# gman90/lime

Hardware: AMD Instinct MI355X
Metric: intervals/sec for pairwise intersect+merge at 1/2/4/8 GPUs; % of HBM peak GB/s (higher is better)
Workload: dtype u32

## Files before the change

### lime_amd/csrc/intersect.hip

```cpp
#include "common.hpp"

namespace lime {

struct PairsPlan {
    lime_ctx *ctx;
    const lime_set *A, *B;
    int64_t threshold;
    int64_t tp;
    bool filtered;
    int64_t a_own, b_own;
    int64_t nt0, nt1;
    uint32_t *olo = nullptr, *ocnt = nullptr;
    uint64_t *toff = nullptr;
    uint32_t *win = nullptr;
    uint32_t *tseg = nullptr;
    int64_t total = 0;
    int tpf = 1;
    const lime_set *A_out = nullptr;
    lime_set *W = nullptr;
    int64_t reach = -1;
};

void intersect_free(PairsPlan *pl);

namespace {

constexpr int IB = 256;
constexpr int OPT = 4;
constexpr int OT = IB * OPT;
constexpr int WCAP = 4096;
constexpr int64_t SBLK = 131072;

typedef uint32_t u32x4 __attribute__((ext_vector_type(4)));

struct StreamArgs {
    const uint32_t *ogs, *oge, *orow;
    const uint32_t *pgs, *pge, *prow;
    const uint32_t *ogs_o, *oge_o, *pgs_o, *pge_o;
    int64_t no, np;
    uint32_t lo_off;
    int zw_skip;
    int64_t reach;
    int64_t tile0;
    int64_t owner0;
};

__device__ __forceinline__ void owner_keys(uint32_t og, uint32_t oe, uint32_t lo_off, int64_t tp,
                                           int64_t &lo_key, int64_t &hi_key) {
    lo_key = (int64_t)og + lo_off;
    hi_key = (int64_t)oe - tp + 1;
}

using dev::wave_lower_bound;

__device__ __forceinline__ uint32_t contig_off(const uint32_t *__restrict__ off, int32_t nc,
                                               uint32_t g) {
    int64_t c = dev::upper_bound(off, 0, (int64_t)nc, g) - 1;
    return off[c < 0 ? 0 : c];
}

__device__ __forceinline__ void wave_lower_bound2(const uint32_t *__restrict__ a, int64_t n,
                                                  int64_t key0, int64_t key1, int64_t &r0,
                                                  int64_t &r1) {
    int64_t lo0 = 0, hi0 = n, lo1 = 0, hi1 = n;
    const int lane = dev::lane_id();
    while (hi0 - lo0 > 64 || hi1 - lo1 > 64) {
        const int64_t st0 = (hi0 - lo0 + 64) / 65, st1 = (hi1 - lo1 + 64) / 65;
        const int64_t i0 = lo0 + st0 * (lane + 1) - 1, i1 = lo1 + st1 * (lane + 1) - 1;
        const bool a0 = hi0 - lo0 > 64 && i0 < hi0;
        const bool a1 = hi1 - lo1 > 64 && i1 < hi1;
        const uint32_t v0 = a0 ? a[i0] : 0u, v1 = a1 ? a[i1] : 0u;
        if (hi0 - lo0 > 64) {
            const int c = __popcll(__ballot(a0 && (int64_t)v0 < key0));
            const int64_t nlo = c == 0 ? lo0 : lo0 + st0 * c;
            hi0 = c == 64 ? hi0 : min(hi0, lo0 + st0 * (c + 1) - 1);
            lo0 = nlo;
        }
        if (hi1 - lo1 > 64) {
            const int c = __popcll(__ballot(a1 && (int64_t)v1 < key1));
            const int64_t nlo = c == 0 ? lo1 : lo1 + st1 * c;
            hi1 = c == 64 ? hi1 : min(hi1, lo1 + st1 * (c + 1) - 1);
            lo1 = nlo;
        }
    }
    const int64_t j0 = lo0 + lane, j1 = lo1 + lane;
    const bool b0 = j0 < hi0, b1 = j1 < hi1;
    const uint32_t v0 = b0 ? a[j0] : 0u, v1 = b1 ? a[j1] : 0u;
    r0 = lo0 + __popcll(__ballot(b0 && (int64_t)v0 < key0));
    r1 = lo1 + __popcll(__ballot(b1 && (int64_t)v1 < key1));
}

__global__ __launch_bounds__(IB) void k_windows(StreamArgs sa, int64_t tp, int64_t ntiles,
                                                uint32_t *__restrict__ win,
                                                const uint32_t *__restrict__ off, int32_t nc,
                                                uint32_t *__restrict__ tseg) {
    const int64_t t = (int64_t)blockIdx.x * (IB / 64) + threadIdx.x / 64;
    if (t >= ntiles) return;
    const int lane = dev::lane_id();
    const int64_t o0 = t * OT;
    const int64_t o1 = min(o0 + OT, sa.no);
    int64_t hmax = INT64_MIN;
    for (int64_t j = o0 + lane; j < o1; j += 64) hmax = max(hmax, (int64_t)sa.oge[j] - tp + 1);
    hmax = dev::wave_reduce_max(hmax);
    const int64_t lkey = (int64_t)sa.ogs[o0] + sa.lo_off;
    const int64_t lkey_last = (int64_t)sa.ogs[o1 - 1] + sa.lo_off;
    if (hmax < lkey_last) hmax = lkey_last;
    int64_t lo, hi;
    wave_lower_bound2(sa.pgs, sa.np, lkey, hmax, lo, hi);
    if (lane == 0) {
        win[2 * (sa.tile0 + t)] = (uint32_t)lo;
        win[2 * (sa.tile0 + t) + 1] = (uint32_t)hi;
    }
    if (tseg) {
        const uint32_t g0 = sa.ogs_o[o0], g1 = sa.ogs_o[o1 - 1];
        uint32_t a, b;
        if (nc <= 64) {
            const uint32_t v = lane < nc ? off[lane] : 0xffffffffu;
            const int c0 = __popcll(__ballot(lane < nc && v <= g0)) - 1;
            const int c1 = __popcll(__ballot(lane < nc && v <= g1)) - 1;
            a = off[c0 < 0 ? 0 : c0];
            b = off[c1 < 0 ? 0 : c1];
        } else {
            a = contig_off(off, nc, g0);
            b = contig_off(off, nc, g1);
        }
        if (lane == 0) tseg[sa.tile0 + t] = a == b ? a : 0xffffffffu;
    }
}

__global__ __launch_bounds__(256) void k_windows_lane(StreamArgs sa, int64_t tp, int64_t ntiles,
                                                      int64_t owmax, uint32_t *__restrict__ win,
                                                      const uint32_t *__restrict__ off, int32_t nc,
                                                      uint32_t *__restrict__ tseg) {
    const int64_t t = (int64_t)blockIdx.x * 256 + threadIdx.x;
    if (t >= ntiles) return;
    const int64_t o0 = t * OT;
    const int64_t o1 = min(o0 + OT, sa.no);
    const uint32_t g0 = sa.ogs[o0], g1 = sa.ogs[o1 - 1];
    const int64_t lkey = (int64_t)g0 + sa.lo_off;
    int64_t hkey = (int64_t)g1 + owmax - tp + 1;
    const int64_t lkey_last = (int64_t)g1 + sa.lo_off;
    if (hkey < lkey_last) hkey = lkey_last;
    int64_t bl = 0, bh = 0;
    const int64_t n = sa.np;
    for (int64_t step = n > 0 ? (int64_t)1 << (63 - __builtin_clzll((uint64_t)n)) : 0; step > 0;
         step >>= 1) {
        const uint32_t vl = bl + step <= n ? sa.pgs[bl + step - 1] : 0xffffffffu;
        const uint32_t vh = bh + step <= n ? sa.pgs[bh + step - 1] : 0xffffffffu;
        if (bl + step <= n && (int64_t)vl < lkey) bl += step;
        if (bh + step <= n && (int64_t)vh < hkey) bh += step;
    }
    win[2 * (sa.tile0 + t)] = (uint32_t)bl;
    win[2 * (sa.tile0 + t) + 1] = (uint32_t)bh;
    if (tseg) {
        const uint32_t a = contig_off(off, nc, sa.ogs_o[o0]), b = contig_off(off, nc, sa.ogs_o[o1 - 1]);
        tseg[sa.tile0 + t] = a == b ? a : 0xffffffffu;
    }
}

template <bool FILTER, bool OFFS>
__global__ __launch_bounds__(IB) void k_count(StreamArgs sa, int64_t tp, int64_t threshold,
                                              const uint32_t *__restrict__ win,
                                              uint32_t *__restrict__ olo,
                                              uint32_t *__restrict__ ocnt,
                                              uint64_t *__restrict__ tcnt,
                                              uint32_t *__restrict__ oflow) {
    __shared__ uint32_t wgs[WCAP];
    __shared__ uint64_t red[IB / 64];
    __shared__ uint32_t scratch[IB / 64 + 1];
    const int64_t t = blockIdx.x;
    const int64_t o0 = t * OT;
    const int64_t o1 = min(o0 + OT, sa.no);
    const uint32_t wlo = win[2 * (sa.tile0 + t)], whi = win[2 * (sa.tile0 + t) + 1];
    const int64_t wlen = (int64_t)whi - wlo;
    const bool in_lds = wlen <= WCAP;
    constexpr int WPT = WCAP / IB;
    uint32_t wv[WPT];
    if (in_lds && wlen > 0) {
#pragma unroll
        for (int k = 0; k < WPT; ++k)
            wv[k] = sa.pgs[wlo + min((int64_t)(k * IB + threadIdx.x), wlen - 1)];
    }
    uint32_t ogv[OPT], oev[OPT];
    static_assert(OPT == 4, "owner loads are one 16-B vector per thread");
    if (o1 - o0 == OT) {
        const uint4 g4 = reinterpret_cast<const uint4 *>(sa.ogs + o0)[threadIdx.x];
        const uint4 e4 = reinterpret_cast<const uint4 *>(sa.oge + o0)[threadIdx.x];
        ogv[0] = g4.x, ogv[1] = g4.y, ogv[2] = g4.z, ogv[3] = g4.w;
        oev[0] = e4.x, oev[1] = e4.y, oev[2] = e4.z, oev[3] = e4.w;
    } else {
#pragma unroll
        for (int k = 0; k < OPT; ++k) {
            const int64_t j = o0 + threadIdx.x * OPT + k;
            ogv[k] = j < o1 ? sa.ogs[j] : 0u;
            oev[k] = j < o1 ? sa.oge[j] : 0u;
        }
    }
    if (in_lds && wlen > 0) {
#pragma unroll
        for (int k = 0; k < WPT; ++k)
            if (k * IB + (int)threadIdx.x < wlen) wgs[k * IB + threadIdx.x] = wv[k];
    }
    __syncthreads();
    int64_t lkv[OPT], hkv[OPT], lov[OPT], hiv[OPT];
#pragma unroll
    for (int k = 0; k < OPT; ++k) owner_keys(ogv[k], oev[k], sa.lo_off, tp, lkv[k], hkv[k]);
    if (in_lds) {
        int64_t key[2 * OPT];
        int b[2 * OPT];
#pragma unroll
        for (int k = 0; k < OPT; ++k) {
            key[k] = lkv[k];
            key[OPT + k] = hkv[k];
        }
        dev::lds_lower_bounds(wgs, (int)wlen, key, b);
#pragma unroll
        for (int k = 0; k < OPT; ++k) {
            lov[k] = wlo + b[k];
            hiv[k] = hkv[k] > lkv[k] ? wlo + b[OPT + k] : lov[k];
        }
    } else {
#pragma unroll
        for (int k = 0; k < OPT; ++k) {
            lov[k] = dev::lower_bound(sa.pgs, (int64_t)wlo, (int64_t)whi, lkv[k]);
            hiv[k] = hkv[k] > lkv[k] ? dev::lower_bound(sa.pgs, lov[k], (int64_t)whi, hkv[k])
                                     : lov[k];
        }
    }
    uint32_t cv[OPT];
    uint64_t csum = 0;
#pragma unroll
    for (int k = 0; k < OPT; ++k) {
        const int64_t j = o0 + threadIdx.x * OPT + k;
        cv[k] = 0;
        if (j >= o1) continue;
        const uint32_t og = ogv[k];
        int64_t lo = lov[k], hi = hiv[k];
        const bool keep0 = sa.reach > 0 && og == 0 && (int64_t)sa.ogs_o[j] < sa.reach;
        if (sa.zw_skip && !keep0) {
            while (lo < whi && sa.pgs[lo] == og && sa.pge[lo] == og) ++lo;
            if (hi < lo) hi = lo;
        }
        if (FILTER) {
            uint32_t c = 0;
            for (int64_t p = lo; p < hi; ++p) c += (int64_t)(sa.pge[p] - sa.pgs[p]) >= threshold;
            cv[k] = c;
        } else {
            cv[k] = (uint32_t)(hi - lo);
        }
        lov[k] = lo;
        csum += cv[k];
    }
    uint32_t run = 0;
    if (OFFS) {
        uint32_t tot;
        run = dev::block_exclusive_sum<IB>((uint32_t)csum, scratch, &tot);
    }
    __syncthreads();
    uint32_t *slo = wgs, *sct = wgs + OT;
#pragma unroll
    for (int k = 0; k < OPT; ++k) {
        slo[threadIdx.x * OPT + k] = (uint32_t)lov[k];
        sct[threadIdx.x * OPT + k] = OFFS ? run : cv[k];
        run += cv[k];
    }
    __syncthreads();
#pragma unroll
    for (int k = 0; k < OPT; ++k) {
        const int q = k * IB + threadIdx.x;
        if (o0 + q < o1) {
            olo[sa.owner0 + o0 + q] = slo[q];
            ocnt[sa.owner0 + o0 + q] = sct[q];
        }
    }
    uint64_t sum = csum;
    sum = dev::wave_reduce_sum(sum);
    if (dev::lane_id() == 0) red[threadIdx.x / 64] = sum;
    __syncthreads();
    if (threadIdx.x == 0) {
        uint64_t s = 0;
        for (int i = 0; i < IB / 64; ++i) s += red[i];
        tcnt[sa.tile0 + t] = s;
        if (s > 0xffffffffull && oflow)
            atomicOr(oflow, 1u);
        else if (s > 0x7fffffffull && oflow)
            atomicOr(oflow, 2u);
    }
}


struct FillArgs {
    StreamArgs s[2];
    const uint32_t *olo, *ocnt;
    const uint64_t *toff;
    const uint32_t *win;
    const uint32_t *tseg;
    int64_t ntiles;
    int64_t total;
    const uint32_t *off;
    int32_t n_contigs;
    int64_t first, count;
    u32x4 *out;
    uint64_t *cksum;
};

constexpr int FB = 512;
constexpr int FW = FB / 64;
#ifndef LIME_FILL_WGS
#define LIME_FILL_WGS 2
#endif
constexpr int PCAP = LIME_FILL_WGS >= 3 ? 1792 : 2048;
constexpr int PCAP2 = 2496;
#ifndef LIME_FILL_SPARSE
#define LIME_FILL_SPARSE 16
#endif
constexpr int64_t GR = 1ll << 40;

template <int TPF> struct FillShape {
    static constexpr int OTF = OT * TPF;
    static constexpr int FOPT = OTF / FB;
    static constexpr int CAP = TPF == 1 ? PCAP : PCAP2;
    static constexpr int PPT = (CAP + FB - 1) / FB;
};

template <int TPF> struct ParWin {
    u32x4 v[PCAP];
    __device__ __forceinline__ void put(int i, uint32_t g, uint32_t e, uint32_t r) {
        v[i] = u32x4{g, e, r, 0u};
    }
    __device__ __forceinline__ u32x4 get(uint32_t i) const { return v[i]; }
};
template <> struct ParWin<2> {
    uint32_t g[PCAP2], e[PCAP2], r[PCAP2];
    __device__ __forceinline__ void put(int i, uint32_t pg, uint32_t pe, uint32_t pr) {
        g[i] = pg;
        e[i] = pe;
        r[i] = pr;
    }
    __device__ __forceinline__ u32x4 get(uint32_t i) const { return u32x4{g[i], e[i], r[i], 0u}; }
};

__device__ __forceinline__ int64_t wave_tile_of(const uint64_t *__restrict__ a, int64_t n,
                                                uint64_t key) {
    int64_t lo = 0, hi = n;
    const int lane = dev::lane_id();
    while (hi - lo > 64) {
        const int64_t step = (hi - lo + 64) / 65;
        const int64_t idx = lo + step * (lane + 1) - 1;
        const bool le = idx < hi && a[idx] <= key;
        const int c = __popcll(__ballot(le));
        const int64_t nlo = c == 0 ? lo : lo + step * c;
        const int64_t nhi = c == 64 ? hi : min(hi, lo + step * (c + 1) - 1);
        lo = nlo;
        hi = nhi;
    }
    const int64_t idx = lo + lane;
    const bool le = idx < hi && a[idx] <= key;
    return lo + __popcll(__ballot(le)) - 1;
}

template <int TPF> struct TileRegs {
    static constexpr int FO = FillShape<TPF>::FOPT, PP = FillShape<TPF>::PPT;
    uint32_t off[FO], lo[FO], og[FO], oe[FO], orw[FO];
    uint32_t pg[PP], pe[PP], pr[PP];
    uint32_t wlo, whi, seg;
    uint64_t tnext;
    int64_t t1;
};

__device__ __forceinline__ int64_t stream0_tiles(const FillArgs &fa) {
    return fa.s[0].tile0 + (fa.s[0].no + OT - 1) / OT;
}

__device__ __forceinline__ int tile_stream(const FillArgs &fa, int64_t t) {
    return t < stream0_tiles(fa) ? 0 : 1;
}

template <int TPF>
__device__ __forceinline__ void tile_load(const FillArgs &fa, int64_t t, TileRegs<TPF> &r,
                                          const uint64_t *toff, const uint32_t *win,
                                          const uint32_t *tseg) {
    constexpr int FO = FillShape<TPF>::FOPT, PP = FillShape<TPF>::PPT;
    const int st = tile_stream(fa, t);
    const StreamArgs sa = st ? fa.s[1] : fa.s[0];
    const int64_t t1 = min(t + TPF, st == 0 ? stream0_tiles(fa) : fa.ntiles);
    const int64_t o0 = (t - sa.tile0) * OT;
    const int nown = (int)min((int64_t)FillShape<TPF>::OTF, sa.no - o0);
    uint32_t add = 0;
    if (TPF > 1) {
        const int u = __builtin_amdgcn_readfirstlane((int)(threadIdx.x / (FB / TPF)));
        if (u > 0 && t + u < t1) add = (uint32_t)(toff[t + u] - toff[t]);
    }
#pragma unroll
    for (int k = 0; k < FO; ++k) {
        const int q = threadIdx.x * FO + k;
        const bool v = q < nown;
        const int64_t j = o0 + q;
        r.off[k] = v ? fa.ocnt[sa.owner0 + j] + add : 0u;
        r.lo[k] = v ? fa.olo[sa.owner0 + j] : 0u;
        r.og[k] = v ? sa.ogs_o[j] : 0u;
        r.oe[k] = v ? sa.oge_o[j] : 0u;
        r.orw[k] = v ? sa.orow[j] : 0u;
    }
    r.wlo = win[2 * t];
    r.whi = win[2 * t + 1];
    r.seg = tseg[t];
    if (TPF > 1 && t1 - 1 > t) {
        r.wlo = min(r.wlo, win[2 * (t1 - 1)]);
        r.whi = max(r.whi, win[2 * (t1 - 1) + 1]);
        if (tseg[t1 - 1] != r.seg) r.seg = 0xffffffffu;
    }
    r.t1 = t1;
    r.tnext = t1 < fa.ntiles ? toff[t1] : (uint64_t)fa.total;
    const int wl = (int)min((int64_t)(r.whi - r.wlo), (int64_t)FillShape<TPF>::CAP);
#pragma unroll
    for (int k = 0; k < PP; ++k) {
        const int i = k * FB + threadIdx.x;
        const bool v = i < wl;
        r.pg[k] = v ? sa.pgs_o[r.wlo + i] : 0u;
        r.pe[k] = v ? sa.pge_o[r.wlo + i] : 0u;
        r.pr[k] = v ? sa.prow[r.wlo + i] : 0u;
    }
}

__device__ __forceinline__ int wave_owner_of(const uint2 *off, int lo, int hi, uint32_t key) {
    const int lane = dev::lane_id();
    while (hi - lo > 64) {
        const int step = (hi - lo + 64) / 65;
        const int idx = lo + step * (lane + 1) - 1;
        const bool le = idx < hi && off[idx].y <= key;
        const int c = __popcll(__ballot(le));
        const int nlo = c == 0 ? lo : lo + step * c;
        hi = c == 64 ? hi : min(hi, lo + step * (c + 1) - 1);
        lo = nlo;
    }
    const int idx = lo + lane;
    const bool le = idx < hi && off[idx].y <= key;
    return lo + __popcll(__ballot(le)) - 1;
}

template <bool LDSP, bool CKSUM, bool WIN, int TPF>
__device__ __forceinline__ void emit(const FillArgs &fa, const StreamArgs &sa, int st,
                                     const uint2 *s_lo_off, const u32x4 *s_own,
                                     const ParWin<TPF> &s_par, uint32_t wlo, int64_t tbase,
                                     int64_t o, int64_t gend, int &q, uint64_t &hsum,
                                     uint64_t &hxor) {
    uint2 lof = s_lo_off[q], nxt = s_lo_off[q + 1];
    u32x4 *out = fa.out + (tbase - fa.first);
    for (; o < gend; o += 64) {
        const uint32_t ou = (uint32_t)o;
        while (nxt.y <= ou) {
            ++q;
            lof = nxt;
            nxt = s_lo_off[q + 1];
        }
        const uint32_t p = lof.x + (ou - lof.y);
        const u32x4 ow = s_own[q];
        u32x4 pa;
        if (LDSP)
            pa = s_par.get(p - wlo);
        else
            pa = u32x4{sa.pgs_o[p], sa.pge_o[p], sa.prow[p], 0u};
        const uint32_t rs =
            (WIN ? (st == 0 ? ow.x : pa.x) : (ow.x > pa.x ? ow.x : pa.x)) - ow.w;
        const uint32_t re =
            (WIN ? (st == 0 ? ow.y : pa.y) : (ow.y < pa.y ? ow.y : pa.y)) - ow.w;
        const uint32_t ar = st == 0 ? ow.z : pa.z;
        const uint32_t br = st == 0 ? pa.z : ow.z;
        if (CKSUM) {
            const uint64_t h = dev::pair_hash(rs, re, ar, br);
            hsum += h;
            hxor ^= h;
        } else {
            out[o] = u32x4{rs, re, ar, br};
        }
    }
}

template <bool LDSP, bool CKSUM, bool WIN, int TPF>
__device__ __forceinline__ void emit_sparse(const FillArgs &fa, const StreamArgs &sa, int st,
                                            const uint2 *s_lo_off, const u32x4 *s_own,
                                            const ParWin<TPF> &s_par, uint32_t wlo, int64_t tbase,
                                            int64_t gb, int64_t gend, int qa, int qmax,
                                            uint32_t *wslot, uint64_t &hsum, uint64_t &hxor) {
    const uint32_t lane = dev::lane_id();
    u32x4 *out = fa.out + (tbase - fa.first);
    for (int64_t ob = gb; ob < gend; ob += 64) {
        const uint32_t o0 = (uint32_t)ob;
        int adv = 0;
        wslot[lane] = 0u;
        for (int qb = qa + 1;; qb += 64) {
            const int qj = qb + (int)lane;
            const uint32_t rel = qj <= qmax ? s_lo_off[qj].y - o0 : 0xffffffffu;
            if (rel < 64u) atomicMax(&wslot[rel], (uint32_t)qj + 1u);
            const uint64_t m = __ballot(rel <= 64u);
            adv += __popcll(m);
            if (m != ~0ull) break;
        }
        const uint32_t mx = dev::wave_inclusive_max(wslot[lane]);
        const int cnt = mx ? (int)mx - 1 - qa : 0;
        const int64_t o = ob + lane;
        if (o < gend) {
            const int q = qa + cnt;
            const uint2 lof = s_lo_off[q];
            const uint32_t ou = (uint32_t)o;
            const uint32_t p = lof.x + (ou - lof.y);
            const u32x4 ow = s_own[q];
            u32x4 pa;
            if (LDSP)
                pa = s_par.get(p - wlo);
            else
                pa = u32x4{sa.pgs_o[p], sa.pge_o[p], sa.prow[p], 0u};
            const uint32_t rs =
                (WIN ? (st == 0 ? ow.x : pa.x) : (ow.x > pa.x ? ow.x : pa.x)) - ow.w;
            const uint32_t re =
                (WIN ? (st == 0 ? ow.y : pa.y) : (ow.y < pa.y ? ow.y : pa.y)) - ow.w;
            const uint32_t ar = st == 0 ? ow.z : pa.z;
            const uint32_t br = st == 0 ? pa.z : ow.z;
            if (CKSUM) {
                const uint64_t h = dev::pair_hash(rs, re, ar, br);
                hsum += h;
                hxor ^= h;
            } else {
                out[o] = u32x4{rs, re, ar, br};
            }
        }
        qa += adv;
    }
}

template <int TPF, bool CKSUM, bool WIN>
__global__ __launch_bounds__(FB, 2 * LIME_FILL_WGS) void k_fill(FillArgs fa, int64_t per, int64_t gran,
                                                               const uint64_t *__restrict__ toff,
                                                               const uint32_t *__restrict__ win,
                                                               const uint32_t *__restrict__ tseg) {
    constexpr int OTF = FillShape<TPF>::OTF, FO = FillShape<TPF>::FOPT,
                  PP = FillShape<TPF>::PPT, CAP = FillShape<TPF>::CAP;
    __shared__ uint2 s_lo_off[OTF + 1];
    __shared__ u32x4 s_own[OTF];
    __shared__ ParWin<TPF> s_par;
    __shared__ uint32_t s_wslot[TPF > 1 ? FW : 1][64];
    __shared__ int64_t s_tile;
    __shared__ uint64_t s_red[2][FW];
    static_assert(sizeof(s_lo_off) + sizeof(s_own) + sizeof(s_par) + sizeof(s_wslot) +
                          sizeof(s_tile) + sizeof(s_red) <= 160 * 1024 / LIME_FILL_WGS,
                  "k_fill's LDS must keep LIME_FILL_WGS workgroups per CU");

    const int64_t ob = fa.first + (int64_t)blockIdx.x * per;
    const int64_t oend = min(fa.first + fa.count, ob + per);
    if (ob >= oend) return;
    const int w = threadIdx.x / 64, lane = dev::lane_id();
    if (w == 0) {
        int64_t t0 = wave_tile_of(fa.toff, fa.ntiles, (uint64_t)ob);
        const int64_t base = t0 < stream0_tiles(fa) ? 0 : stream0_tiles(fa);
        t0 = base + (t0 - base) / TPF * TPF;
        if (lane == 0) s_tile = t0;
    }
    __syncthreads();
    int64_t t = dev::uni64(s_tile);
    uint64_t hsum = 0, hxor = 0;
    TileRegs<TPF> R;
    tile_load<TPF>(fa, t, R, toff, win, tseg);
    while (true) {
        const int st = tile_stream(fa, t);
        const StreamArgs sa = st ? fa.s[1] : fa.s[0];
        const int64_t o0 = (t - sa.tile0) * OT;
        const int nown = (int)min((int64_t)OTF, sa.no - o0);
        const int64_t tbase = (int64_t)toff[t];
        const int64_t tn = dev::uni64(R.t1);
        const uint32_t ttot = (uint32_t)(R.tnext - (uint64_t)tbase);
#pragma unroll
        for (int k = 0; k < FO; ++k) {
            const int q = threadIdx.x * FO + k;
            if (q < nown) {
                const uint32_t sg =
                    R.seg != 0xffffffffu ? R.seg : contig_off(fa.off, fa.n_contigs, R.og[k]);
                s_own[q] = u32x4{R.og[k], R.oe[k], R.orw[k], sg};
            }
            s_lo_off[q] = make_uint2(R.lo[k], q < nown ? R.off[k] : ttot);
        }
        if (threadIdx.x == 0) s_lo_off[OTF] = make_uint2(0u, ttot);
        const uint32_t wlo = R.wlo, whi = R.whi;
        const bool par_lds = (int64_t)whi - wlo <= CAP;
        if (par_lds) {
#pragma unroll
            for (int k = 0; k < PP; ++k) {
                const int i = k * FB + threadIdx.x;
                if (i < (int)(whi - wlo)) s_par.put(i, R.pg[k], R.pe[k], R.pr[k]);
            }
        }
        __syncthreads();
        const bool more = tn < fa.ntiles && (int64_t)R.tnext < oend;
        if (more) tile_load<TPF>(fa, tn, R, toff, win, tseg);
        const int64_t lb = max(ob - tbase, (int64_t)0);
        const int64_t le = min(oend - tbase, (int64_t)ttot);
        const int64_t rounds = max((int64_t)1, (le - lb + FW * gran - 1) / (FW * gran));
        const int64_t gsz = (((le - lb + FW * rounds - 1) / (FW * rounds)) + 63) & ~(int64_t)63;
        int qw = 0;
        for (int64_t gb = lb + (int64_t)w * gsz; gb < le; gb += (int64_t)FW * gsz) {
            const int64_t gend = min(le, gb + gsz);
            int64_t o = gb + lane;
            qw = wave_owner_of(s_lo_off, qw, nown, (uint32_t)gb);
            int q = qw;
            if (TPF > 1) {
                uint32_t *wslot = s_wslot[TPF > 1 ? w : 0];
                if (par_lds)
                    emit_sparse<true, CKSUM, WIN, TPF>(fa, sa, st, s_lo_off, s_own, s_par, wlo,
                                                       tbase, gb, gend, qw, OTF, wslot, hsum,
                                                       hxor);
                else
                    emit_sparse<false, CKSUM, WIN, TPF>(fa, sa, st, s_lo_off, s_own, s_par, wlo,
                                                        tbase, gb, gend, qw, OTF, wslot, hsum,
                                                        hxor);
            } else if (par_lds)
                emit<true, CKSUM, WIN, TPF>(fa, sa, st, s_lo_off, s_own, s_par, wlo, tbase, o,
                                            gend, q, hsum, hxor);
            else
                emit<false, CKSUM, WIN, TPF>(fa, sa, st, s_lo_off, s_own, s_par, wlo, tbase, o,
                                             gend, q, hsum, hxor);
        }
        __syncthreads();
        if (!more) break;
        t = tn;
    }
    if (CKSUM) {
        hsum = dev::wave_reduce_sum(hsum);
        uint64_t x = hxor;
        x = dev::wave_reduce_xor(x);
        if (lane == 0) {
            s_red[0][w] = hsum;
            s_red[1][w] = x;
        }
        __syncthreads();
        if (threadIdx.x == 0) {
            uint64_t a = 0, b = 0;
            for (int i = 0; i < FW; ++i) {
                a += s_red[0][i];
                b ^= s_red[1][i];
            }
            atomicAdd((unsigned long long *)&fa.cksum[0], (unsigned long long)a);
            atomicXor((unsigned long long *)&fa.cksum[1], (unsigned long long)b);
        }
    }
}

template <bool CKSUM>
__global__ __launch_bounds__(IB) void k_fill_filtered(FillArgs fa, int64_t threshold) {
    __shared__ uint32_t scratch[IB / 64 + 1];
    __shared__ uint64_t s_red[2][IB / 64];
    const int64_t t = blockIdx.x;
    const int st = t < fa.s[0].tile0 + (fa.s[0].no + OT - 1) / OT ? 0 : 1;
    const StreamArgs sa = st ? fa.s[1] : fa.s[0];
    const int64_t lt = t - sa.tile0;
    const int64_t o0 = lt * OT;
    const int nown = (int)min((int64_t)OT, sa.no - o0);
    const int64_t tbase = (int64_t)fa.toff[t];
    uint32_t c[OPT];
    uint32_t csum = 0;
#pragma unroll
    for (int k = 0; k < OPT; ++k) {
        const int q = threadIdx.x * OPT + k;
        c[k] = q < nown ? fa.ocnt[sa.owner0 + o0 + q] : 0u;
        csum += c[k];
    }
    uint32_t ttot;
    int64_t pos = tbase + dev::block_exclusive_sum<IB>(csum, scratch, &ttot);
    uint64_t hsum = 0, hxor = 0;
    const int64_t wend = fa.first + fa.count;
    for (int k = 0; k < OPT; ++k) {
        const int q = threadIdx.x * OPT + k;
        if (q >= nown || c[k] == 0) continue;
        if (pos + c[k] <= fa.first || pos >= wend) {
            pos += c[k];
            continue;
        }
        const int64_t j = o0 + q;
        const uint32_t og = sa.ogs[j], oe = sa.oge[j], orow = sa.orow[j];
        const uint32_t sg = contig_off(fa.off, fa.n_contigs, og);
        uint32_t p = fa.olo[sa.owner0 + j];
        uint32_t left = c[k];
        for (; left > 0; ++p) {
            const uint32_t pg = sa.pgs[p], pe = sa.pge[p];
            if ((int64_t)(pe - pg) < threshold) continue;
            --left;
            if (pos >= fa.first && pos < wend) {
                const uint32_t pr = sa.prow[p];
                const uint32_t rs = (og > pg ? og : pg) - sg;
                const uint32_t re = (oe < pe ? oe : pe) - sg;
                const uint32_t ar = st == 0 ? orow : pr;
                const uint32_t br = st == 0 ? pr : orow;
                if (CKSUM) {
                    uint64_t h = dev::pair_hash(rs, re, ar, br);
                    hsum += h;
                    hxor ^= h;
                } else {
                    u32x4 v = {rs, re, ar, br};
                    fa.out[pos - fa.first] = v;
                }
            }
            ++pos;
        }
    }
    if (CKSUM) {
        hsum = dev::wave_reduce_sum(hsum);
        uint64_t x = hxor;
        x = dev::wave_reduce_xor(x);
        if (dev::lane_id() == 0) {
            s_red[0][threadIdx.x / 64] = hsum;
            s_red[1][threadIdx.x / 64] = x;
        }
        __syncthreads();
        if (threadIdx.x == 0) {
            uint64_t a = 0, b = 0;
            for (int i = 0; i < IB / 64; ++i) {
                a += s_red[0][i];
                b ^= s_red[1][i];
            }
            atomicAdd((unsigned long long *)&fa.cksum[0], (unsigned long long)a);
            atomicXor((unsigned long long *)&fa.cksum[1], (unsigned long long)b);
        }
    }
}

constexpr int64_t WLANE_MAX = 65536;
void launch_windows(lime_ctx *ctx, const StreamArgs &sa, int64_t tp, int64_t ntl, int64_t owmax,
                    uint32_t *win, const uint32_t *off, int32_t nc, uint32_t *tseg) {
    if (owmax <= WLANE_MAX)
        hipLaunchKernelGGL(k_windows_lane, dim3(blocks_for(ntl, 256)), dim3(256), 0, S(ctx), sa, tp,
                           ntl, owmax, win, off, nc, tseg);
    else
        hipLaunchKernelGGL(k_windows, dim3(blocks_for(ntl, IB / 64)), dim3(IB), 0, S(ctx), sa, tp,
                           ntl, win, off, nc, tseg);
}

StreamArgs stream_args(const lime_set *O, const lime_set *P, int st, int64_t threshold,
                       int64_t tile0, int64_t owner0, int64_t n_own = -1,
                       const lime_set *O_out = nullptr, const lime_set *P_out = nullptr,
                       int64_t reach = -1) {
    StreamArgs s;
    if (!O_out) O_out = O;
    if (!P_out) P_out = P;
    s.ogs = O->gs;
    s.oge = O->ge;
    s.orow = O->row;
    s.pgs = P->gs;
    s.pge = P->ge;
    s.prow = P->row;
    s.ogs_o = O_out->gs;
    s.oge_o = O_out->ge;
    s.pgs_o = P_out->gs;
    s.pge_o = P_out->ge;
    s.no = n_own >= 0 ? n_own : O->n;
    s.np = P->n;
    s.lo_off = st == 0 ? 0u : 1u;
    s.zw_skip = (st == 0 && threshold <= 0 && P->has_zero_width) ? 1 : 0;
    s.reach = st == 0 ? reach : -1;
    s.tile0 = tile0;
    s.owner0 = owner0;
    return s;
}

FillArgs fill_args(PairsPlan *pl) {
    FillArgs fa;
    fa.s[0] = stream_args(pl->A, pl->B, 0, pl->threshold, 0, 0, pl->a_own, pl->A_out, nullptr,
                          pl->reach);
    fa.s[1] = stream_args(pl->B, pl->A, 1, pl->threshold, pl->nt0, pl->a_own, pl->b_own, nullptr,
                          pl->A_out);
    fa.olo = pl->olo;
    fa.ocnt = pl->ocnt;
    fa.toff = pl->toff;
    fa.win = pl->win;
    fa.tseg = pl->tseg;
    fa.total = pl->total;
    fa.ntiles = pl->nt0 + pl->nt1;
    fa.off = pl->A->d_off;
    fa.n_contigs = pl->A->n_contigs;
    fa.first = 0;
    fa.count = 0;
    fa.out = nullptr;
    fa.cksum = nullptr;
    return fa;
}

int64_t fill_span(int64_t count) {
    static const int64_t slots = [] {
        int dev = 0, cus = 256, occ = 2;
        (void)hipGetDevice(&dev);
        (void)hipDeviceGetAttribute(&cus, hipDeviceAttributeMultiprocessorCount, dev);
        (void)hipOccupancyMaxActiveBlocksPerMultiprocessor(&occ, k_fill<1, false, false>, FB, 0);
        return (int64_t)cus * (occ > 0 ? occ : 1);
    }();
    int64_t per = (count + slots - 1) / slots;
    per = (per + 63) & ~(int64_t)63;
    return per < 4096 ? 4096 : per;
}

template <int TPF>
void launch_k_fill(lime_ctx *ctx, dim3 g, const FillArgs &fa, int64_t per, bool cksum, bool win) {
    if (cksum && win)
        hipLaunchKernelGGL((k_fill<TPF, true, true>), g, dim3(FB), 0, S(ctx), fa, per, (int64_t)GR,
                           fa.toff, fa.win, fa.tseg);
    else if (cksum)
        hipLaunchKernelGGL((k_fill<TPF, true, false>), g, dim3(FB), 0, S(ctx), fa, per, (int64_t)GR,
                           fa.toff, fa.win, fa.tseg);
    else if (win)
        hipLaunchKernelGGL((k_fill<TPF, false, true>), g, dim3(FB), 0, S(ctx), fa, per, (int64_t)GR,
                           fa.toff, fa.win, fa.tseg);
    else
        hipLaunchKernelGGL((k_fill<TPF, false, false>), g, dim3(FB), 0, S(ctx), fa, per,
                           (int64_t)GR, fa.toff, fa.win, fa.tseg);
}

int launch_fill(PairsPlan *pl, int64_t first, int64_t count, u32x4 *out, uint64_t *cksum) {
    lime_ctx *ctx = pl->ctx;
    if (count <= 0) return LIME_OK;
    FillArgs fa = fill_args(pl);
    fa.first = first;
    fa.count = count;
    fa.out = out;
    fa.cksum = cksum;
    if (pl->filtered) {
        const unsigned grid = (unsigned)(pl->nt0 + pl->nt1);
        if (cksum)
            hipLaunchKernelGGL(k_fill_filtered<true>, dim3(grid), dim3(IB), 0, S(ctx), fa,
                               pl->threshold);
        else
            hipLaunchKernelGGL(k_fill_filtered<false>, dim3(grid), dim3(IB), 0, S(ctx), fa,
                               pl->threshold);
    } else {
        const int64_t per = fill_span(count);
        const int64_t grid = (count + per - 1) / per;
        if (grid > 0x7fffffff) return fail(LIME_ERR_OVERFLOW, "fill window too large");
        const dim3 g((unsigned)grid);
        const bool win = pl->reach >= 0;
        if (pl->tpf == 2)
            launch_k_fill<2>(ctx, g, fa, per, cksum != nullptr, win);
        else
            launch_k_fill<1>(ctx, g, fa, per, cksum != nullptr, win);
    }
    LIME_HIP(hipGetLastError());
    return LIME_OK;
}

__global__ __launch_bounds__(256) void k_widen(const uint32_t *__restrict__ gs,
                                               const uint32_t *__restrict__ ge, int64_t n,
                                               int64_t d, const uint32_t *__restrict__ off,
                                               int32_t nc, uint32_t *__restrict__ ws,
                                               uint32_t *__restrict__ we) {
    const int64_t i = (int64_t)blockIdx.x * 256 + threadIdx.x;
    if (i >= n) return;
    const uint32_t g = gs[i];
    int64_t c = dev::upper_bound(off, 0, (int64_t)nc, g) - 1;
    if (c < 0) c = 0;
    const int64_t lo = c == 0 ? 0 : (int64_t)off[c] - 1;
    const int64_t hi = (int64_t)off[c + 1];
    const int64_t s = (int64_t)g - d, e = (int64_t)ge[i] + d;
    ws[i] = (uint32_t)(s > lo ? s : lo);
    we[i] = (uint32_t)(e < hi ? e : hi);
}

}

int intersect_plan(lime_ctx *ctx, const lime_set *A, const lime_set *B, int64_t threshold,
                   int64_t a_own, int64_t b_own, PairsPlan **out, const lime_set *A_out,
                   int64_t reach) {
    if (a_own < 0 || a_own > A->n) a_own = A->n;
    if (b_own < 0 || b_own > B->n) b_own = B->n;
    PairsPlan *pl = new PairsPlan();
    pl->ctx = ctx;
    pl->A = A;
    pl->B = B;
    pl->A_out = A_out;
    pl->reach = reach;
    pl->a_own = a_own;
    pl->b_own = b_own;
    pl->threshold = threshold;
    pl->tp = threshold > 1 ? threshold : 1;
    pl->filtered = threshold >= 1 && (int64_t)std::min(A->min_width, B->min_width) < threshold &&
                   A->n > 0 && B->n > 0;
    pl->nt0 = (a_own + OT - 1) / OT;
    pl->nt1 = (b_own + OT - 1) / OT;
    const int64_t nt = pl->nt0 + pl->nt1;
    int rc = LIME_OK;
    uint64_t *tcnt = nullptr, *total = nullptr;
    if ((rc = alloc(ctx, &pl->olo, (size_t)(a_own + b_own))) ||
        (rc = alloc(ctx, &pl->ocnt, (size_t)(a_own + b_own))) ||
        (rc = alloc(ctx, &pl->toff, (size_t)nt)) || (rc = alloc(ctx, &pl->win, (size_t)2 * nt)) ||
        (rc = alloc(ctx, &pl->tseg, (size_t)nt)) ||
        (rc = alloc(ctx, &tcnt, (size_t)nt)) || (rc = alloc(ctx, &total, 2))) {
        delete pl;
        return rc;
    }
    uint32_t *oflow = reinterpret_cast<uint32_t *>(total + 1);
    LIME_HIP(hipMemsetAsync(total + 1, 0, sizeof(uint64_t), S(ctx)));
    if (A->n > 0 && B->n > 0) {
        for (int st = 0; st < 2; ++st) {
            const lime_set *O = st == 0 ? A : B;
            const lime_set *P = st == 0 ? B : A;
            const int64_t ntl = st == 0 ? pl->nt0 : pl->nt1;
            StreamArgs sa = stream_args(O, P, st, threshold, st == 0 ? 0 : pl->nt0,
                                        st == 0 ? 0 : a_own, st == 0 ? a_own : b_own,
                                        st == 0 ? A_out : nullptr, st == 0 ? nullptr : A_out,
                                        reach);
            if (ntl == 0) continue;
            const int64_t owmax = (int64_t)O->max_width + (st == 0 && reach > 0 ? 2 * reach : 0);
            launch_windows(ctx, sa, pl->tp, ntl, owmax, pl->win, (const uint32_t *)O->d_off,
                           O->n_contigs, pl->tseg);
            if (pl->filtered)
                hipLaunchKernelGGL((k_count<true, false>), dim3((unsigned)ntl), dim3(IB), 0, S(ctx), sa,
                                   pl->tp, threshold, (const uint32_t *)pl->win, pl->olo, pl->ocnt,
                                   tcnt, oflow);
            else
                hipLaunchKernelGGL((k_count<false, true>), dim3((unsigned)ntl), dim3(IB), 0, S(ctx), sa,
                                   pl->tp, threshold, (const uint32_t *)pl->win, pl->olo, pl->ocnt,
                                   tcnt, oflow);
            LIME_HIP(hipGetLastError());
        }
    } else {
        LIME_HIP(hipMemsetAsync(tcnt, 0, sizeof(uint64_t) * (size_t)(nt > 0 ? nt : 1), S(ctx)));
        LIME_HIP(hipMemsetAsync(pl->ocnt, 0,
                                sizeof(uint32_t) * (size_t)(a_own + b_own > 0 ? a_own + b_own : 1),
                                S(ctx)));
    }
    LIME_TRY(scan_exclusive_u64(ctx, tcnt, pl->toff, nt, total));
    uint64_t tot[2] = {0, 0};
    LIME_TRY(read_back(ctx, tot, total, sizeof(tot)));
    release(ctx, tcnt);
    release(ctx, total);
    if (tot[1] & 1) {
        intersect_free(pl);
        return fail(LIME_ERR_OVERFLOW,
                    "a tile of 1024 owner rows has 2^32 or more candidate pairs (pile-up)");
    }
    pl->total = (int64_t)tot[0];
    pl->tpf = !(tot[1] & 2) && pl->total < (int64_t)LIME_FILL_SPARSE * (a_own + b_own) ? 2 : 1;
    *out = pl;
    return LIME_OK;
}

int owner_ranges(lime_ctx *ctx, const lime_set *O, const lime_set *P, int st, int64_t threshold,
                 uint32_t *olo, uint32_t *ocnt) {
    if (O->n == 0) return LIME_OK;
    if (P->n == 0) {
        LIME_HIP(hipMemsetAsync(olo, 0, sizeof(uint32_t) * (size_t)O->n, S(ctx)));
        LIME_HIP(hipMemsetAsync(ocnt, 0, sizeof(uint32_t) * (size_t)O->n, S(ctx)));
        return LIME_OK;
    }
    const int64_t tp = threshold > 1 ? threshold : 1;
    const int64_t ntl = (O->n + OT - 1) / OT;
    uint32_t *win;
    uint64_t *tcnt;
    LIME_TRY(alloc(ctx, &win, (size_t)2 * ntl));
    LIME_TRY(alloc(ctx, &tcnt, (size_t)ntl));
    StreamArgs sa = stream_args(O, P, st, threshold, 0, 0);
    launch_windows(ctx, sa, tp, ntl, (int64_t)O->max_width, win, nullptr, 0, nullptr);
    hipLaunchKernelGGL((k_count<false, false>), dim3((unsigned)ntl), dim3(IB), 0, S(ctx), sa, tp,
                       threshold,
                       (const uint32_t *)win, olo, ocnt, tcnt, (uint32_t *)nullptr);
    LIME_HIP(hipGetLastError());
    release(ctx, win);
    release(ctx, tcnt);
    return LIME_OK;
}

int intersect_fill(PairsPlan *pl, int64_t first, int64_t count, lime_pair *d_out) {
    if (first < 0 || count < 0 || first + count > pl->total)
        return fail(LIME_ERR_ARG, "fill window outside [0, n_pairs)");
    return launch_fill(pl, first, count, reinterpret_cast<u32x4 *>(d_out), nullptr);
}

int intersect_checksum(PairsPlan *pl, uint64_t *sum, uint64_t *xr) {
    lime_ctx *ctx = pl->ctx;
    uint64_t *ck;
    LIME_TRY(alloc(ctx, &ck, 2));
    LIME_HIP(hipMemsetAsync(ck, 0, 16, S(ctx)));
    const int64_t step = (int64_t)SBLK * 1048576;
    for (int64_t f = 0; f < pl->total; f += step)
        LIME_TRY(launch_fill(pl, f, std::min(step, pl->total - f), nullptr, ck));
    uint64_t h[2];
    LIME_TRY(read_back(ctx, h, ck, 16));
    release(ctx, ck);
    *sum = h[0];
    *xr = h[1];
    return LIME_OK;
}

int64_t plan_total(const PairsPlan *pl) { return pl->total; }

int window_plan(lime_ctx *ctx, const lime_set *A, const lime_set *B, int64_t d,
                PairsPlan **out) {
    if (d < 1) return intersect_plan(ctx, A, B, 0, -1, -1, out, A, 0);
    lime_set *W = new lime_set();
    W->ctx = ctx;
    W->n = A->n;
    W->row = A->row;
    W->d_off = A->d_off;
    W->space_keep = A->space_keep;
    W->n_contigs = A->n_contigs;
    W->off = A->off;
    W->len = A->len;
    W->min_width = A->min_width;
    W->max_width = A->max_width;
    W->has_zero_width = false;
    int rc = LIME_OK;
    if ((rc = alloc(ctx, &W->gs, (size_t)std::max<int64_t>(A->n, 1))) ||
        (rc = alloc(ctx, &W->ge, (size_t)std::max<int64_t>(A->n, 1)))) {
        release(ctx, W->gs);
        delete W;
        return rc;
    }
    if (A->n > 0) {
        hipLaunchKernelGGL(k_widen, dim3(blocks_for(A->n, 256)), dim3(256), 0, S(ctx), A->gs,
                           A->ge, A->n, d, (const uint32_t *)A->d_off, A->n_contigs, W->gs,
                           W->ge);
        LIME_HIP(hipGetLastError());
    }
    PairsPlan *pl = nullptr;
    rc = intersect_plan(ctx, W, B, 0, -1, -1, &pl, A, d);
    if (rc != LIME_OK) {
        release(ctx, W->gs);
        release(ctx, W->ge);
        delete W;
        return rc;
    }
    pl->W = W;
    *out = pl;
    return LIME_OK;
}

void intersect_free(PairsPlan *pl) {
    lime_ctx *ctx = pl->ctx;
    if (pl->W) {
        release(ctx, pl->W->gs);
        release(ctx, pl->W->ge);
        delete pl->W;
    }
    release(ctx, pl->olo);
    release(ctx, pl->ocnt);
    release(ctx, pl->toff);
    release(ctx, pl->win);
    release(ctx, pl->tseg);
    delete pl;
}

}
```

Baseline: 3.773 billion.

## Pack per-owner window offset and count into one word for small tiles

When a tile's search window fits in 12 bits and its total pair count fits in 20 bits, k_count stores the window-relative lo and the running offset in a single 32-bit word and skips the separate ocnt write. A per-tile format byte records which layout was used, and the fill kernel decodes packed tiles instead of loading ocnt. This cuts one 4-byte global store per owner in count and one 4-byte load per owner in fill. In exchange it adds a format array, a branch per tile, and decode arithmetic.

```diff
diff --git a/lime_amd/csrc/intersect.hip b/lime_amd/csrc/intersect.hip
--- a/lime_amd/csrc/intersect.hip
+++ b/lime_amd/csrc/intersect.hip
@@ -11,6 +11,7 @@
     int64_t a_own, b_own;
     int64_t nt0, nt1;
     uint32_t *olo = nullptr, *ocnt = nullptr;
+    uint8_t *tfmt = nullptr;
     uint64_t *toff = nullptr;
     uint32_t *win = nullptr;
     uint32_t *tseg = nullptr;
@@ -30,6 +31,13 @@
 constexpr int OT = IB * OPT;
 constexpr int WCAP = 4096;
 constexpr int64_t SBLK = 131072;
+#ifndef LIME_COUNT_PACK
+#define LIME_COUNT_PACK 1
+#endif
+constexpr int PK_OBITS = 20, PK_LBITS = 32 - PK_OBITS;
+constexpr int64_t PK_WMAX = (1 << PK_LBITS) - 1;
+constexpr uint32_t PK_OMASK = (1u << PK_OBITS) - 1;
+static_assert(PK_WMAX <= WCAP, "a packed tile's window is searched in LDS");
 
 typedef uint32_t u32x4 __attribute__((ext_vector_type(4)));
 
@@ -164,7 +172,8 @@
                                               uint32_t *__restrict__ olo,
                                               uint32_t *__restrict__ ocnt,
                                               uint64_t *__restrict__ tcnt,
-                                              uint32_t *__restrict__ oflow) {
+                                              uint32_t *__restrict__ oflow,
+                                              uint8_t *__restrict__ tfmt) {
     __shared__ uint32_t wgs[WCAP];
     __shared__ uint64_t red[IB / 64];
     __shared__ uint32_t scratch[IB / 64 + 1];
@@ -252,17 +261,27 @@
         csum += cv[k];
     }
     uint32_t run = 0;
+    bool packed = false;
     if (OFFS) {
         uint32_t tot;
         run = dev::block_exclusive_sum<IB>((uint32_t)csum, scratch, &tot);
+        packed = LIME_COUNT_PACK && wlen <= PK_WMAX && tot <= PK_OMASK;
     }
     __syncthreads();
     uint32_t *slo = wgs, *sct = wgs + OT;
-#pragma unroll
-    for (int k = 0; k < OPT; ++k) {
-        slo[threadIdx.x * OPT + k] = (uint32_t)lov[k];
-        sct[threadIdx.x * OPT + k] = OFFS ? run : cv[k];
-        run += cv[k];
+    if (packed) {
+#pragma unroll
+        for (int k = 0; k < OPT; ++k) {
+            slo[threadIdx.x * OPT + k] = (uint32_t)(lov[k] - wlo) << PK_OBITS | run;
+            run += cv[k];
+        }
+    } else {
+#pragma unroll
+        for (int k = 0; k < OPT; ++k) {
+            slo[threadIdx.x * OPT + k] = (uint32_t)lov[k];
+            sct[threadIdx.x * OPT + k] = OFFS ? run : cv[k];
+            run += cv[k];
+        }
     }
     __syncthreads();
 #pragma unroll
@@ -270,7 +289,7 @@
         const int q = k * IB + threadIdx.x;
         if (o0 + q < o1) {
             olo[sa.owner0 + o0 + q] = slo[q];
-            ocnt[sa.owner0 + o0 + q] = sct[q];
+            if (!packed) ocnt[sa.owner0 + o0 + q] = sct[q];
         }
     }
     uint64_t sum = csum;
@@ -281,6 +300,7 @@
         uint64_t s = 0;
         for (int i = 0; i < IB / 64; ++i) s += red[i];
         tcnt[sa.tile0 + t] = s;
+        if (OFFS) tfmt[sa.tile0 + t] = packed ? 1 : 0;
         if (s > 0xffffffffull && oflow)
             atomicOr(oflow, 1u);
         else if (s > 0x7fffffffull && oflow)
@@ -295,6 +315,7 @@
     const uint64_t *toff;
     const uint32_t *win;
     const uint32_t *tseg;
+    const uint8_t *tfmt;
     int64_t ntiles;
     int64_t total;
     const uint32_t *off;
@@ -366,7 +387,14 @@
     uint32_t wlo, whi, seg;
     uint64_t tnext;
     int64_t t1;
+    bool pk;
+    uint32_t pwlo, padd;
 };
+
+__device__ __forceinline__ bool tile_packed(const uint8_t *tfmt, int64_t t) {
+    const uint32_t w = reinterpret_cast<const uint32_t *>(tfmt)[t >> 2];
+    return (w >> (8 * (uint32_t)(t & 3))) & 1u;
+}
 
 __device__ __forceinline__ int64_t stream0_tiles(const FillArgs &fa) {
     return fa.s[0].tile0 + (fa.s[0].no + OT - 1) / OT;
@@ -379,7 +407,7 @@
 template <int TPF>
 __device__ __forceinline__ void tile_load(const FillArgs &fa, int64_t t, TileRegs<TPF> &r,
                                           const uint64_t *toff, const uint32_t *win,
-                                          const uint32_t *tseg) {
+                                          const uint32_t *tseg, const uint8_t *tfmt) {
     constexpr int FO = FillShape<TPF>::FOPT, PP = FillShape<TPF>::PPT;
     const int st = tile_stream(fa, t);
     const StreamArgs sa = st ? fa.s[1] : fa.s[0];
@@ -387,23 +415,36 @@
     const int64_t o0 = (t - sa.tile0) * OT;
     const int nown = (int)min((int64_t)FillShape<TPF>::OTF, sa.no - o0);
     uint32_t add = 0;
+    int64_t tu = t;
     if (TPF > 1) {
         const int u = __builtin_amdgcn_readfirstlane((int)(threadIdx.x / (FB / TPF)));
-        if (u > 0 && t + u < t1) add = (uint32_t)(toff[t + u] - toff[t]);
-    }
+        if (u > 0 && t + u < t1) {
+            add = (uint32_t)(toff[t + u] - toff[t]);
+            tu = t + u;
+        }
+    }
+    r.pk = LIME_COUNT_PACK && tile_packed(tfmt, tu);
+    r.padd = add;
 #pragma unroll
     for (int k = 0; k < FO; ++k) {
         const int q = threadIdx.x * FO + k;
         const bool v = q < nown;
         const int64_t j = o0 + q;
-        r.off[k] = v ? fa.ocnt[sa.owner0 + j] + add : 0u;
         r.lo[k] = v ? fa.olo[sa.owner0 + j] : 0u;
         r.og[k] = v ? sa.ogs_o[j] : 0u;
         r.oe[k] = v ? sa.oge_o[j] : 0u;
         r.orw[k] = v ? sa.orow[j] : 0u;
     }
+    if (!r.pk) {
+#pragma unroll
+        for (int k = 0; k < FO; ++k) {
+            const int q = threadIdx.x * FO + k;
+            r.off[k] = q < nown ? fa.ocnt[sa.owner0 + o0 + q] + add : 0u;
+        }
+    }
     r.wlo = win[2 * t];
     r.whi = win[2 * t + 1];
+    r.pwlo = TPF > 1 ? win[2 * tu] : r.wlo;
     r.seg = tseg[t];
     if (TPF > 1 && t1 - 1 > t) {
         r.wlo = min(r.wlo, win[2 * (t1 - 1)]);
@@ -533,7 +574,8 @@
 __global__ __launch_bounds__(FB, 2 * LIME_FILL_WGS) void k_fill(FillArgs fa, int64_t per, int64_t gran,
                                                                const uint64_t *__restrict__ toff,
                                                                const uint32_t *__restrict__ win,
-                                                               const uint32_t *__restrict__ tseg) {
+                                                               const uint32_t *__restrict__ tseg,
+                                                               const uint8_t *__restrict__ tfmt) {
     constexpr int OTF = FillShape<TPF>::OTF, FO = FillShape<TPF>::FOPT,
                   PP = FillShape<TPF>::PPT, CAP = FillShape<TPF>::CAP;
     __shared__ uint2 s_lo_off[OTF + 1];
@@ -560,7 +602,7 @@
     int64_t t = dev::uni64(s_tile);
     uint64_t hsum = 0, hxor = 0;
     TileRegs<TPF> R;
-    tile_load<TPF>(fa, t, R, toff, win, tseg);
+    tile_load<TPF>(fa, t, R, toff, win, tseg, tfmt);
     while (true) {
         const int st = tile_stream(fa, t);
         const StreamArgs sa = st ? fa.s[1] : fa.s[0];
@@ -577,7 +619,12 @@
                     R.seg != 0xffffffffu ? R.seg : contig_off(fa.off, fa.n_contigs, R.og[k]);
                 s_own[q] = u32x4{R.og[k], R.oe[k], R.orw[k], sg};
             }
-            s_lo_off[q] = make_uint2(R.lo[k], q < nown ? R.off[k] : ttot);
+            uint32_t lo = R.lo[k], off = R.off[k];
+            if (LIME_COUNT_PACK && R.pk) {
+                off = (lo & PK_OMASK) + R.padd;
+                lo = R.pwlo + (lo >> PK_OBITS);
+            }
+            s_lo_off[q] = make_uint2(lo, q < nown ? off : ttot);
         }
         if (threadIdx.x == 0) s_lo_off[OTF] = make_uint2(0u, ttot);
         const uint32_t wlo = R.wlo, whi = R.whi;
@@ -591,7 +638,7 @@
         }
         __syncthreads();
         const bool more = tn < fa.ntiles && (int64_t)R.tnext < oend;
-        if (more) tile_load<TPF>(fa, tn, R, toff, win, tseg);
+        if (more) tile_load<TPF>(fa, tn, R, toff, win, tseg, tfmt);
         const int64_t lb = max(ob - tbase, (int64_t)0);
         const int64_t le = min(oend - tbase, (int64_t)ttot);
         const int64_t rounds = max((int64_t)1, (le - lb + FW * gran - 1) / (FW * gran));
@@ -771,6 +818,7 @@
     fa.toff = pl->toff;
     fa.win = pl->win;
     fa.tseg = pl->tseg;
+    fa.tfmt = pl->tfmt;
     fa.total = pl->total;
     fa.ntiles = pl->nt0 + pl->nt1;
     fa.off = pl->A->d_off;
@@ -799,16 +847,16 @@
 void launch_k_fill(lime_ctx *ctx, dim3 g, const FillArgs &fa, int64_t per, bool cksum, bool win) {
     if (cksum && win)
         hipLaunchKernelGGL((k_fill<TPF, true, true>), g, dim3(FB), 0, S(ctx), fa, per, (int64_t)GR,
-                           fa.toff, fa.win, fa.tseg);
+                           fa.toff, fa.win, fa.tseg, fa.tfmt);
     else if (cksum)
         hipLaunchKernelGGL((k_fill<TPF, true, false>), g, dim3(FB), 0, S(ctx), fa, per, (int64_t)GR,
-                           fa.toff, fa.win, fa.tseg);
+                           fa.toff, fa.win, fa.tseg, fa.tfmt);
     else if (win)
         hipLaunchKernelGGL((k_fill<TPF, false, true>), g, dim3(FB), 0, S(ctx), fa, per, (int64_t)GR,
-                           fa.toff, fa.win, fa.tseg);
+                           fa.toff, fa.win, fa.tseg, fa.tfmt);
     else
         hipLaunchKernelGGL((k_fill<TPF, false, false>), g, dim3(FB), 0, S(ctx), fa, per,
-                           (int64_t)GR, fa.toff, fa.win, fa.tseg);
+                           (int64_t)GR, fa.toff, fa.win, fa.tseg, fa.tfmt);
 }
 
 int launch_fill(PairsPlan *pl, int64_t first, int64_t count, u32x4 *out, uint64_t *cksum) {
@@ -887,6 +935,7 @@
         (rc = alloc(ctx, &pl->ocnt, (size_t)(a_own + b_own))) ||
         (rc = alloc(ctx, &pl->toff, (size_t)nt)) || (rc = alloc(ctx, &pl->win, (size_t)2 * nt)) ||
         (rc = alloc(ctx, &pl->tseg, (size_t)nt)) ||
+        (rc = alloc(ctx, &pl->tfmt, ((size_t)nt + 3) & ~(size_t)3)) ||
         (rc = alloc(ctx, &tcnt, (size_t)nt)) || (rc = alloc(ctx, &total, 2))) {
         delete pl;
         return rc;
@@ -909,11 +958,11 @@
             if (pl->filtered)
                 hipLaunchKernelGGL((k_count<true, false>), dim3((unsigned)ntl), dim3(IB), 0, S(ctx), sa,
                                    pl->tp, threshold, (const uint32_t *)pl->win, pl->olo, pl->ocnt,
-                                   tcnt, oflow);
+                                   tcnt, oflow, pl->tfmt);
             else
                 hipLaunchKernelGGL((k_count<false, true>), dim3((unsigned)ntl), dim3(IB), 0, S(ctx), sa,
                                    pl->tp, threshold, (const uint32_t *)pl->win, pl->olo, pl->ocnt,
-                                   tcnt, oflow);
+                                   tcnt, oflow, pl->tfmt);
             LIME_HIP(hipGetLastError());
         }
     } else {
@@ -956,7 +1005,8 @@
     launch_windows(ctx, sa, tp, ntl, (int64_t)O->max_width, win, nullptr, 0, nullptr);
     hipLaunchKernelGGL((k_count<false, false>), dim3((unsigned)ntl), dim3(IB), 0, S(ctx), sa, tp,
                        threshold,
-                       (const uint32_t *)win, olo, ocnt, tcnt, (uint32_t *)nullptr);
+                       (const uint32_t *)win, olo, ocnt, tcnt, (uint32_t *)nullptr,
+                       (uint8_t *)nullptr);
     LIME_HIP(hipGetLastError());
     release(ctx, win);
     release(ctx, tcnt);
@@ -1040,6 +1090,7 @@
     release(ctx, pl->toff);
     release(ctx, pl->win);
     release(ctx, pl->tseg);
+    release(ctx, pl->tfmt);
     delete pl;
 }
 
```

Result: slower. 3.589 billion (-4.9%).
